# guoyihonggyh/MOBODY-Model-Based-Off-Dynamics-Offline-Reinforcement-Learning

Hardware: AMD Instinct MI355X
Metric: transitions/sec (minibatch rows through train(), refresh amortised at 1/5000) + grad-steps/sec (higher is better)
Workload: dtype f16x2

## Files before the change

### mobody-model-based-off-dynamics-offline-reinforcement-learning_amd/csrc/mlp_bwd.hip

```cpp
#include <stdlib.h>

#include "common.h"
#include "layers_bf.h"
#include "train.h"

namespace mobody {

template <int MT, int MASK>
struct MaskPre {
  uint32_t w[MASK == 1 ? MT : 1][2];
  float v[MASK == 1 ? 1 : MT][2][MASK == 1 ? 1 : 16];
};
template <int MT, int MASK>
__device__ __forceinline__ void mask_fetch(MaskPre<MT, MASK>& p, const float* __restrict__ h, const uint32_t* __restrict__ bits,
                                           int rows_here) {
  const int lane = lane_id(), w = wave_id(), i = lane & 31, hh = lane >> 5;
  if constexpr (MASK == 1) {
#pragma unroll
    for (int mt = 0; mt < MT; ++mt) {
      const int g = min(mt, (rows_here + 31) / 32 - 1);
      p.w[mt][0] = bits[g * HID + 64 * w + i]; p.w[mt][1] = bits[g * HID + 64 * w + 32 + i];
    }
  } else {
    const float* hp = h + 64 * w + i;
// ... 4 lines not shown
        const int row = min(32 * mt + (r & 3) + 8 * (r >> 2) + 4 * hh, rows_here - 1);
        p.v[mt][0][r] = hp[row * HID];
        p.v[mt][1][r] = hp[row * HID + 32];
      }
  }
}

template <int MT, int MASK>
__device__ __forceinline__ float wide_mask_apply(f32x16 (&acc)[MT][2], const MaskPre<MT, MASK>& pre, int rows_here, float prescale) {
  const int hh = lane_id() >> 5;
  constexpr bool BITS = MASK == 1;
  const auto& hv = pre.v;
  const auto& mw = pre.w;
  float mx = 0.f;
  f32x16 pa[MT][2];
#pragma unroll
  for (int mt = 0; mt < MT; ++mt) { pa[mt][0] = acc[mt][0] * prescale; pa[mt][1] = acc[mt][1] * prescale; }
  auto sweep = [&](auto guarded) {
#pragma unroll
    for (int mt = 0; mt < MT; ++mt)
#pragma unroll
      for (int nt = 0; nt < 2; ++nt)
#pragma unroll
        for (int r = 0; r < 16; ++r) {
          const int rb = (r & 3) + 8 * (r >> 2) + 4 * hh;
          const bool valid = !decltype(guarded)::value || 32 * mt + rb < rows_here;
          const float a = pa[mt][nt][r];
          float dz;
          if constexpr (MASK == 2) {
            dz = valid ? a * hv[mt][nt][r] : 0.f;
          } else {
            bool on;
            if constexpr (BITS) on = (mw[mt][nt] >> rb) & 1u;
            else on = hv[mt][nt][r] > 0.f;
            dz = (on && valid) ? a : 0.f;
          }
          acc[mt][nt][r] = dz;
          mx = fmaxf(mx, fabsf(dz));
        }
  };
  if (rows_here == 32 * MT) sweep(std::false_type{});
  else sweep(std::true_type{});
  return finite_tile_max<MT>(acc, mx);
}

template <int MT, int PM>
__device__ __forceinline__ void wide_store_colsum(f32x16 (&acc)[MT][2], float* Xs, float* gdst, int rows_here, int e,
                                                  float (&cs)[2], const PlaneSave& gs = PlaneSave{nullptr, 0, nullptr}) {
  const int lane = lane_id(), w = wave_id();
  const int i = lane & 31, hh = lane >> 5;
  cs[0] = cs[1] = 0.f;
  if constexpr (PM > 0) {
    const float sc = Split<PM>::F16 ? exp2i(e) : 1.f;
    if (gs.base != nullptr && (int)threadIdx.x < MT) gs.e_out[threadIdx.x] = e;
#pragma unroll
    for (int mt = 0; mt < MT; ++mt)
#pragma unroll
      for (int nt = 0; nt < 2; ++nt) {
        const f32x16 ys = Split<PM>::F16 ? acc[mt][nt] * sc : acc[mt][nt];
#pragma unroll
        for (int g = 0; g < 4; ++g) {
          float y4[4];
#pragma unroll
          for (int j = 0; j < 4; ++j) y4[j] = ys[4 * g + j];
          planes_store4<PM, 32 * MT>(reinterpret_cast<char*>(Xs), 64 * w + 32 * nt + i, 8 * mt + 2 * g + hh, y4, gs.base, gs.plane_stride);
        }
      }
  }
#pragma unroll
  for (int mt = 0; mt < MT; ++mt)
#pragma unroll
    for (int nt = 0; nt < 2; ++nt)
#pragma unroll
      for (int r = 0; r < 16; ++r) {
        const float dz = acc[mt][nt][r];
        if constexpr (PM == 0) Xs[(32 * mt + (r & 3) + 8 * (r >> 2) + 4 * hh) * LDX + 64 * w + 32 * nt + i] = dz;
        cs[nt] += dz;
      }
  if (gdst != nullptr) wide_store_rows<MT>(acc, gdst, rows_here);
  cs[0] += __shfl_xor(cs[0], 32);
  cs[1] += __shfl_xor(cs[1], 32);
}

__device__ __forceinline__ void bwd_seed(const Mlp3BwdArgs& a, float* Xs, float* red, int m, long long row0, int rows_here,
                                         int TB) {
  const BwdSeed& sd = a.seed;
  const int Np3 = a.Np3;
  const int t = threadIdx.x;
  float l0 = 0.f, l1 = 0.f;
  if (sd.mode == 1 || sd.mode == 2) {
    if (t < TB) {
      const bool ok = t < rows_here;
      const long long row = row0 + (ok ? t : 0);
      float v = 0.f;
      if (sd.mode == 1) {
        const float qn = sd.qnext ? sd.qnext[row] : fminf(sd.qt[row], sd.qt[a.rows + row]);
        const float y = sd.r[row] + sd.nd[row] * sd.gamma * qn;
        const float d = sd.q[(long long)m * a.rows + row] - y;
        v = ok ? 2.f * d * sd.inv_ng : 0.f;
        l0 = ok ? d * d : 0.f;
      } else {
        const ActorRowArgs& r = sd.ar;
        const float q0 = r.qp[row], q1 = r.qp[r.N + row];
        const float c = -policy_weight(r) / (float)r.Ng;
        const float g0 = q0 < q1 ? 1.f : (q0 == q1 ? 0.5f : 0.f);
        v = ok ? c * (m == 0 ? g0 : 1.f - g0) : 0.f;
        if (m == 0 && ok && row < r.Nt) r.bcw[row] = bc_weight(r, row);
      }
      Xs[t] = v;
      if (sd.dz3_out != nullptr && ok) {
        float* g = sd.dz3_out + ((long long)m * a.rows + row) * Np3;
        g[0] = v;
        for (int c = 1; c < Np3; ++c) g[c] = 0.f;
      }
    }
  } else {
    const ActorRowArgs& r = sd.ar;
    const float wscale = r.h.bc_coef * 2.f / ((float)r.Ntg * (float)r.A);
    for (int e = t; e < TB * Np3; e += NTHREADS) {
      const int rr = e / Np3, j = e - rr * Np3;
      const bool ok = rr < rows_here && j < r.A;
      const long long row = row0 + (rr < rows_here ? rr : 0);
      const int jc = j < r.A ? j : 0;
      const bool bc = row < r.Nt;
      const float p = r.pi[row * r.A + jc];
      const float d0 = r.dxa[row * r.A + jc], d1 = r.dxa[(r.N + row) * r.A + jc];
      const float act = r.act[row * r.A + jc];
      const float w = r.bcw[bc ? row : 0];
      float v = 0.f;
      if (ok) {
        float d = d0 + d1;
        if (bc) { const float df = p - act; d += wscale * w * df; l1 += w * (df * df); }
        const float th = p / r.h.max_action;
        v = d * r.h.max_action * (1.f - th * th);
        if (j == 0) l0 = l0 - fminf(r.qp[row], r.qp[r.N + row]);
      }
      Xs[rr * LDX + j] = v;
      if (rr < rows_here) sd.dz3_out[(row0 + rr) * Np3 + j] = v;
    }
  }
  if (sd.mode == 2) return;
#pragma unroll
  for (int o = 32; o > 0; o >>= 1) { l0 += __shfl_xor(l0, o); l1 += __shfl_xor(l1, o); }
  if ((t & 63) == 0) { red[t >> 6] = l0; red[4 + (t >> 6)] = l1; }
  lds_barrier();
  if (t == 0) {
    l0 = red[0] + red[1] + red[2] + red[3];
    l1 = red[4] + red[5] + red[6] + red[7];
    if (sd.mode == 1) sd.lossp[blockIdx.x * 2 + m] = l0;
    else { sd.lossp[2 * blockIdx.x] = l0; sd.lossp[2 * blockIdx.x + 1] = l1; }
  }
}

template <bool DX, int NT, int MASK, int PM = 0>
__global__ __launch_bounds__(NTHREADS, MASK == 1 ? 3 : 2) void k_mlp3_bwd(Mlp3BwdArgs a) {
  constexpr bool BITS = MASK == 1;
  __shared__ float red[8];
  extern __shared__ __attribute__((aligned(16))) float Xs[];
  constexpr int TB = MLP_TILE_ROWS, MT = MLP_MT;
  constexpr int PMX = PM > 0 ? PM : 1;
  const int m = blockIdx.y;
  const long long row0 = (long long)blockIdx.x * TB;
  const int rows_here = (int)min((long long)TB, a.rows - row0);
  const int lane = lane_id(), w = wave_id();
  const float* w3t = a.wt + m * a.t_mstride + a.w3t;
  const float* w2t = a.wt + m * a.t_mstride + a.w2t;
  const float* w1t = a.wt + m * a.t_mstride + a.w1t;
  const float* h1 = BITS ? nullptr : a.h1 + ((long long)m * a.rows + row0) * HID;
  const float* h2 = BITS ? nullptr : a.h2 + ((long long)m * a.rows + row0) * HID;
  const long long mtile = ((long long)m * cdiv(a.rows, 32) + row0 / 32) * HID;
  const uint32_t* m1 = BITS ? a.m1 + mtile : nullptr;
  const uint32_t* m2 = BITS ? a.m2 + mtile : nullptr;
  float* dz2 = a.dz2 ? a.dz2 + ((long long)m * a.rows + row0) * HID : nullptr;
  float* dz1 = a.dz1 ? a.dz1 + ((long long)m * a.rows + row0) * HID : nullptr;
  float* dbp = a.dbp + ((long long)blockIdx.x * gridDim.y + m) * (2 * HID + a.Np3);
  float* scr = reinterpret_cast<float*>(reinterpret_cast<char*>(Xs) + split_scr_offset<PMX, TB>());

  TR(0);
  MaskPre<MT, MASK> mk1, mk2;
  mask_fetch<MT, MASK>(mk2, h2, m2, rows_here);
  if constexpr (BITS) mask_fetch<MT, MASK>(mk1, h1, m1, rows_here);
  WideRingT<(PM > 0 ? 3 : WIDE_RING)> ring;
  const int mode = a.seed.mode;
  const bool rank1 = mode == 1 || mode == 2, with_db = mode != 2;
  const int c0 = (64 * w + (lane & 31)) * 4;
  const float w3c[2] = {w3t[c0], w3t[c0 + 128]};
  if (!rank1) wide_prefetch(w3t, a.Np3, ring);
  if (mode == 0) tile_load(Xs, 0, a.dz3 + ((long long)m * a.rows + row0) * a.Np3, a.Np3, a.Np3, 0, rows_here, TB);
  else bwd_seed(a, Xs, red, m, row0, rows_here, TB);
  lds_barrier();
  TR(1);
  if (with_db && (int)threadIdx.x < a.Np3) {
    float s = 0.f;
    if (!rank1) for (int r = 0; r < TB; ++r) s += Xs[r * LDX + threadIdx.x];
    else if (threadIdx.x == 0) for (int r = 0; r < TB; ++r) s += Xs[r];
    dbp[2 * HID + threadIdx.x] = s;
  }

  f32x16 acc[MT][2];
  float cs[2];
  if (rank1) {
    const int hh = lane >> 5;
#pragma unroll
    for (int mt = 0; mt < MT; ++mt)
#pragma unroll
      for (int g = 0; g < 4; ++g) {
        const f32x4 sv = *reinterpret_cast<const f32x4*>(Xs + 32 * mt + 8 * g + 4 * hh);
#pragma unroll
        for (int j = 0; j < 4; ++j) { acc[mt][0][4 * g + j] = sv[j] * w3c[0]; acc[mt][1][4 * g + j] = sv[j] * w3c[1]; }
      }
  } else {
    wide_zero<MT>(acc);
    wide_gemm<MT>(Xs, w3t, a.Np3, acc, ring);
  }
  TR(2);
  BfRing<PMX> bring;
  const s16x8* w2tp = PM > 0 ? reinterpret_cast<const s16x8*>(a.w2t_planes + m * a.planes_ms) : nullptr;
  if constexpr (PM > 0) bf_prefetch<PMX>(w2tp, bring);
  else wide_prefetch(w2t, HID, ring);
  int e2 = 0;
  {
    const float mx = wide_mask_apply<MT, MASK>(acc, mk2, rows_here, 1.f);
    if constexpr (PM == 4) f16_tile_max_put(mx, scr);
  }
  lds_barrier();
  if constexpr (PM == 4) e2 = f16_scale_exp(f16_tile_max_get(scr));
  PlaneSave gs{nullptr, 0, nullptr};
  if (PM == 4 && a.dz2p != nullptr) {
    gs.base = reinterpret_cast<short*>(a.dz2p) + m * a.dz2p_ms + (row0 / 8) * (HID * 8);
    gs.plane_stride = a.dz2p_plane;
    gs.e_out = a.e2_out + (long long)m * cdiv(a.rows, 32) + row0 / 32;
  }
  wide_store_colsum<MT, PM>(acc, Xs, dz2, rows_here, e2, cs, gs);
  if (with_db && lane < 32) { dbp[HID + 64 * w + lane] = cs[0]; dbp[HID + 64 * w + 32 + lane] = cs[1]; }
  lds_barrier();
  TR(3);
  if constexpr (!BITS) mask_fetch<MT, MASK>(mk1, h1, m1, rows_here);
  wide_zero<MT>(acc);
  if constexpr (PM > 0) bf_gemm<MT, PMX, TB>(reinterpret_cast<const char*>(Xs), w2tp, acc, bring);
  else wide_gemm<MT>(Xs, w2t, HID, acc, ring);
  TR(4);
  NarrowRegs<(NT > 0 ? NT : 1)> br;
  if constexpr (DX && NT > 0) narrow_prefetch<NT>(w1t, 16 * NT, br);
  wide_mask_apply<MT, MASK>(acc, mk1, rows_here, PM == 4 ? exp2i(-(e2 + F16_WSHIFT)) : 1.f);
  lds_barrier();
  wide_store_colsum<MT, 0>(acc, Xs, dz1, rows_here, 0, cs);
  if (with_db && lane < 32) { dbp[64 * w + lane] = cs[0]; dbp[64 * w + 32 + lane] = cs[1]; }
  TR(5);
  if constexpr (DX) {
    lds_barrier();
    float* dx = a.dx + ((long long)m * a.rows + row0) * a.dx_n;
    auto emit = [&](int row, int col, float v) {
      const int c = col - a.dx_c0;
      if (row < rows_here && c >= 0 && c < a.dx_n) dx[row * a.dx_n + c] = v;
    };
    if constexpr (NT > 0) narrow_run<TB / 16, NT>(Xs, br, emit);
    else narrow_layer(Xs, w1t, HID, a.Np1t, emit, TB);
  }
  TR(6);
}

template <bool DX, int NT, int BITS, int NPL = 0>
static int launch_bwd_t(const Mlp3BwdArgs& a, int members, hipStream_t st) {
  constexpr size_t lds = split_lds_bytes<(NPL > 0 ? NPL : 1), MLP_TILE_ROWS>();
  static bool once = false;
  if (!once) {
    int rc = allow_big_lds(k_mlp3_bwd<DX, NT, BITS, NPL>, lds);
    if (rc) return rc;
    once = true;
  }
  dim3 grid((unsigned)cdiv(a.rows, MLP_TILE_ROWS), (unsigned)members);
  ProfScope prof(PROF_MLP_BWD, st);
  hipLaunchKernelGGL((k_mlp3_bwd<DX, NT, BITS, NPL>), grid, dim3(NTHREADS), lds, st, a);
  MB_LAUNCH_OK("k_mlp3_bwd");
  return 0;
}

template <int NPL>
static int launch_bwd_bf(const Mlp3BwdArgs& a, int members, bool with_dx, hipStream_t st) {
  const int nt = a.Np1t == 16 ? 1 : a.Np1t == 32 ? 2 : 0;
  if (!with_dx) return launch_bwd_t<false, 0, 1, NPL>(a, members, st);
  return nt == 1 ? launch_bwd_t<true, 1, 1, NPL>(a, members, st) : nt == 2 ? launch_bwd_t<true, 2, 1, NPL>(a, members, st)
                                                                             : launch_bwd_t<true, 0, 1, NPL>(a, members, st);
}

template <int BITS>
static int launch_bwd_masks(const Mlp3BwdArgs& a, int members, bool with_dx, hipStream_t st) {
  const int nt = a.Np1t == 16 ? 1 : a.Np1t == 32 ? 2 : 0;
  if (!with_dx) return launch_bwd_t<false, 0, BITS>(a, members, st);
  return nt == 1 ? launch_bwd_t<true, 1, BITS>(a, members, st) : nt == 2 ? launch_bwd_t<true, 2, BITS>(a, members, st)
                                                                          : launch_bwd_t<true, 0, BITS>(a, members, st);
}

static int launch_bwd_swish(const Mlp3BwdArgs& a, int members, bool with_dx, hipStream_t st) {
  const int nt = a.Np1t == 16 ? 1 : a.Np1t == 32 ? 2 : 0;
  if (a.prec == PREC_F16X2 && a.w2t_planes != nullptr) {
    if (!with_dx) return launch_bwd_t<false, 0, 2, 4>(a, members, st);
    return nt == 1 ? launch_bwd_t<true, 1, 2, 4>(a, members, st) : nt == 2 ? launch_bwd_t<true, 2, 2, 4>(a, members, st)
                                                                             : launch_bwd_t<true, 0, 2, 4>(a, members, st);
  }
  if (!with_dx) return launch_bwd_t<false, 0, 2>(a, members, st);
  return nt == 1 ? launch_bwd_t<true, 1, 2>(a, members, st) : nt == 2 ? launch_bwd_t<true, 2, 2>(a, members, st)
                                                                         : launch_bwd_t<true, 0, 2>(a, members, st);
}

int launch_mlp3_bwd(const Mlp3BwdArgs& a, int members, bool with_dx, hipStream_t st) {
  if (a.rows <= 0) return 0;
  if (a.swish) return launch_bwd_swish(a, members, with_dx, st);
  if (a.prec != PREC_F32 && a.w2t_planes != nullptr && a.m1 != nullptr && a.m2 != nullptr)
    return a.prec == PREC_BF16 ? launch_bwd_bf<1>(a, members, with_dx, st) : a.prec == PREC_BF16X2 ? launch_bwd_bf<2>(a, members, with_dx, st)
         : a.prec == PREC_BF16X3 ? launch_bwd_bf<3>(a, members, with_dx, st) : launch_bwd_bf<4>(a, members, with_dx, st);
  return a.m1 != nullptr && a.m2 != nullptr ? launch_bwd_masks<1>(a, members, with_dx, st)
                                            : launch_bwd_masks<0>(a, members, with_dx, st);
}

__device__ __forceinline__ __amdgpu_buffer_rsrc_t slice_rsrc(const float* p, int nrows, int ld) {
  return __builtin_amdgcn_make_buffer_rsrc(const_cast<float*>(p), 0, (int)((unsigned)nrows * (unsigned)ld * 4u), 0x00020000);
}
__device__ __forceinline__ float buf_ld(__amdgpu_buffer_rsrc_t r, unsigned voff, unsigned soff) {
  return __builtin_bit_cast(float, __builtin_amdgcn_raw_buffer_load_b32(r, (int)voff, (int)soff, 0));
}

template <int MT, int NT>
__device__ __forceinline__ void wgrad_store(const WgradJob& jb, const WgradArgs& a, f32x16 (&acc)[MT][NT], int k0, int n0,
                                            int slice, int m, float* red) {
  constexpr int TK = 32 * MT, TN = 32 * NT;
  const int lane = lane_id(), w = wave_id();
  const int i = lane & 31, h = lane >> 5;
  float* mine = red + (w & 1) * (TK * TN);
  auto sweep = [&](bool add) {
#pragma unroll
    for (int x = 0; x < MT; ++x)
#pragma unroll
      for (int y = 0; y < NT; ++y)
#pragma unroll
        for (int r = 0; r < 16; ++r) {
          const int kk = 32 * x + (r & 3) + 8 * (r >> 2) + 4 * h;
          float* p = mine + kk * TN + 32 * y + i;
          *p = add ? *p + acc[x][y][r] : acc[x][y][r];
        }
  };
  if (w < 2) sweep(false);
  lds_barrier();
  if (w >= 2) sweep(true);
  lds_barrier();
  float* slab = a.slabs + (long long)slice * a.slab_stride + jb.out_off + m * a.out_mstride;
  if ((jb.wide || jb.transposed) && (jb.out_k & 3) == 0 && (!jb.transposed || (jb.out_ld & 3) == 0)) {
    for (int g = threadIdx.x; g < (TK / 4) * TN; g += NTHREADS) {
      const int kg = g / TN, nn = g - kg * TN;
      f32x4 s;
#pragma unroll
      for (int c = 0; c < 4; ++c) { const int idx = (4 * kg + c) * TN + nn; s[c] = red[idx] + red[TK * TN + idx]; }
      const int gk = k0 + 4 * kg, gn = n0 + nn;
      if (gk < jb.out_k && gn < jb.out_n)
        *reinterpret_cast<f32x4*>(slab + (jb.transposed ? (long long)gn * jb.out_ld + gk : wide_idx(gk, gn))) = s;
    }
    return;
  }
  for (int idx = threadIdx.x; idx < TK * TN; idx += NTHREADS) {
    const int kk = idx / TN, nn = idx - kk * TN;
    const float s = red[idx] + red[TK * TN + idx];
    const int gk = k0 + kk, gn = n0 + nn;
    if (gk < jb.out_k && gn < jb.out_n) {
      if (jb.transposed) slab[(long long)gn * jb.out_ld + gk] = s;
      else if (jb.wide) slab[wide_idx(gk, gn)] = s;
      else slab[(long long)gk * jb.out_ld + gn] = s;
    }
  }
}

template <int MT>
__device__ __forceinline__ void wgrad_tile(const WgradJob& jb, const WgradArgs& a, int tile, int slice, int m, float* red) {
  constexpr int NT = 2, TK = 32 * MT, TN = 32 * NT, U = 4, RB = 2 * U;
  const int lane = lane_id(), w = __builtin_amdgcn_readfirstlane(wave_id());
  const int i = lane & 31, h = lane >> 5;
  const int tk = tile / jb.tiles_n, tn = tile - tk * jb.tiles_n;
  const int k0 = tk * TK, n0 = tn * TN;
  const long long r_begin = ((long long)slice * 4 + w) * a.rows_per_wave;
  const long long r_end = min(a.rows, r_begin + a.rows_per_wave);
  const int lda = jb.lda, ldb = jb.ldb;

  f32x16 acc[MT][NT];
#pragma unroll
  for (int x = 0; x < MT; ++x)
#pragma unroll
    for (int y = 0; y < NT; ++y)
#pragma unroll
      for (int r = 0; r < 16; ++r) acc[x][y][r] = 0.f;

  unsigned oa[MT], ob[NT];
#pragma unroll
  for (int x = 0; x < MT; ++x) { const int c = k0 + 32 * x + i; oa[x] = 4u * (unsigned)((c < jb.ka ? c : 0) + h * lda); }
#pragma unroll
  for (int y = 0; y < NT; ++y) { const int c = n0 + 32 * y + i; ob[y] = 4u * (unsigned)((c < jb.nb ? c : 0) + h * ldb); }

  auto mma = [&](float (&av)[U][MT], float (&bv)[U][NT]) {
// ... 424 lines not shown
```

### mobody-model-based-off-dynamics-offline-reinforcement-learning_amd/csrc/train.h

```cpp
#pragma once
#include <math.h>
#include <stdlib.h>

#include "common.h"
#include "tile.h"
#include "tile_bf.h"
#include "health.h"

namespace mobody {

struct ActorRowArgs {
  const float *qp, *qb, *stats, *pi, *act, *dxa;
  const float* v_true;
  float* bcw;
  long long N, Nt, Ng, Ntg;
  int A;
  MobodyHyper h;
};
__device__ __forceinline__ float policy_weight(const ActorRowArgs& a) {
  return a.h.scale_q ? a.h.weight / (a.stats[0] / (float)a.Ng) : 1.f;
}
__device__ __forceinline__ float bc_weight(const ActorRowArgs& a, long long row) {
  if (!a.h.q_weighted) return 1.f;
  const float qb = fminf(a.qb[row], a.qb[a.Nt + row]);
  const float adv = a.v_true ? qb - a.v_true[row]
                             : qb / (a.stats[1] / (float)a.Ntg);
  return fminf(expf(3.f * adv), 100.f);
}

struct BwdSeed {
  int mode;
  const float *q, *qt, *qnext, *r, *nd;
  float gamma, inv_ng;
  ActorRowArgs ar;
  float* dz3_out;
  float* lossp;
};

struct Mlp3BwdArgs {
  BwdSeed seed;
  const float* dz3;
  const float* h1;
  const float* h2;
  int swish;
  const uint32_t* m1;
  const uint32_t* m2;
  const float* wt;
  const unsigned short* w2t_planes;
  long long planes_ms;
  int prec;
  long long t_mstride, w3t, w2t, w1t;
  int Np3, Np1t;
  long long rows;
  float* dz2;
  float* dz1;
  unsigned short* dz2p;
  long long dz2p_ms;
  long long dz2p_plane;
  int* e2_out;
  float* dbp;
  float* dx;
  int dx_c0, dx_n;
};
int launch_mlp3_bwd(const Mlp3BwdArgs& a, int members, bool with_dx, hipStream_t st);

inline Mlp3BwdArgs bwd_net(const MobodyMlpLayout& L, const float* blob_T, long long rows) {
  Mlp3BwdArgs b{};
  b.wt = blob_T; b.t_mstride = L.t_member_floats;
  b.w3t = L.w3t; b.w2t = L.w2t; b.w1t = L.w1t; b.Np3 = L.Np3; b.Np1t = L.Np1t; b.rows = rows;
  return b;
}
inline void bwd_set_planes(Mlp3BwdArgs& b, const MobodyMlpLayout& L, int prec) {
  b.prec = prec; b.w2t_planes = reinterpret_cast<const unsigned short*>(b.wt + L.w2tp); b.planes_ms = 2 * L.t_member_floats;
}
inline void bwd_set_acts(Mlp3BwdArgs& b, const float* h1, const float* h2, const uint32_t* m1, const uint32_t* m2, int swish) {
  b.h1 = h1; b.h2 = h2; b.m1 = m1; b.m2 = m2; b.swish = swish;
}
inline void bwd_set_grads(Mlp3BwdArgs& b, const float* dz3, float* dz2, float* dz1, float* dbp, int* e2 = nullptr) {
  if (e2 != nullptr && dz2 != nullptr) {
    const long long r32 = (b.rows + 31) & ~31LL;
    b.dz2p = reinterpret_cast<unsigned short*>(dz2); b.dz2p_plane = r32 * HID; b.dz2p_ms = 2 * r32 * HID; b.e2_out = e2;
    dz2 = nullptr;
  }
  b.dz3 = dz3; b.dz2 = dz2; b.dz1 = dz1; b.dbp = dbp;
}

struct WgradJob {
  const float* A; long long a_mstride; int lda, ka;
  const float* B; long long b_mstride; int ldb, nb;
  long long out_off; int out_ld, out_k, out_n;
  int transposed;
  int wide;
  int tiles_n, ntiles;
};
struct WgradArgs {
  const int *eA, *eB;
  long long e_mstride, plane_stride;
  WgradJob job[3];
  long long rows, rows_per_wave;
  float* slabs; long long slab_stride, out_mstride;
  int nsplit, members, tiles_total;
  float* bc_out; const long long* bc_t; float bc_lr;
  int prec;
};
int launch_wgrad(WgradArgs a, hipStream_t st);

struct AdamConsts { float step_size, bc2_sqrt, tau, one_minus_tau, gscale; };
constexpr float ADAM_W1 = (float)(1.0 - 0.9), ADAM_B2 = (float)0.999, ADAM_W2 = (float)(1.0 - 0.999), ADAM_EPS = 1e-8f;

__device__ __forceinline__ void write_w2_planes(float* t_member, const MobodyMlpLayout& L, int k, int n, float w, int precision) {
  short* p2 = reinterpret_cast<short*>(t_member + L.w2p);
  short* p2t = reinterpret_cast<short*>(t_member + L.w2tp);
  if (precision == 4) {
    short t[2];
    split_terms<4>(w * exp2i(F16_WSHIFT), t);
#pragma unroll
    for (int p = 0; p < 2; ++p) { p2[bf_plane_idx(p, k, n)] = t[p]; p2t[bf_plane_idx(p, n, k)] = t[p]; }
  } else {
    short t[3];
    split_terms<3>(w, t);
#pragma unroll
    for (int p = 0; p < 3; ++p) { p2[bf_plane_idx(p, k, n)] = t[p]; p2t[bf_plane_idx(p, n, k)] = t[p]; }
  }
}

__device__ __forceinline__ long long t_blob_index(const MobodyMlpLayout& L, long long o) {
  if (o < L.b1) {
    const long long g = o >> 2;
    const int k = (int)(g / HID) * 4 + (int)(o & 3), n = (int)(g % HID);
    return L.w1t + (long long)n * L.Np1t + k;
  }
  if (o >= L.w2 && o < L.b2) {
    const long long oo = o - L.w2, g = oo >> 2;
    const int k = (int)(g / HID) * 4 + (int)(oo & 3), n = (int)(g % HID);
    return L.w2t + wide_idx(n, k);
  }
  if (o >= L.w3 && o < L.b3) {
    const long long oo = o - L.w3;
    const int k = (int)(oo / L.Np3), n3 = (int)(oo % L.Np3);
    return L.w3t + wide_idx(n3, k);
  }
  return -1;
}

struct AdamTarget {
  float *p, *m, *v, *target, *blob_T;
  float* target_T;
// ... 129 lines not shown
```

### mobody-model-based-off-dynamics-offline-reinforcement-learning_amd/csrc/train.hip

```cpp
#include <math.h>

#include "common.h"
#include "layers.h"
#include "train.h"

namespace mobody {

struct TrainWs {
  uint32_t *mq1, *mq2, *ma1, *ma2;
  int *eh1q, *eh1a, *edz2;
  float *pin;
  float *pi, *qt, *q, *qb, *xq, *h1q, *h2q, *xa, *h1a, *h2a, *dz3q, *dz2, *dz1, *dz3a, *dxa, *bcw, *dbp, *slabs, *lossp;
  float *bc;
  long long total;
  int nsplit_q, nsplit_a, ntiles;
  MobodyMlpLayout Lq, La;
};

static int carve(const MobodyTrainDims& d, float* base, TrainWs& w) {
  int rc = mobody_mlp_layout(d.S + d.A, 1, 2, &w.Lq);
  if (rc) return rc;
  rc = mobody_mlp_layout(d.S, d.A, 1, &w.La);
  if (rc) return rc;
  const long long N = d.N, Nt = d.Nt;
  const long long N32 = (N + 31) & ~31LL;
  long long off = 0;
  auto take = [&](long long n) { float* p = base ? base + off : nullptr; off += (n + 3) & ~3LL; return p; };
  w.pi = take(N * d.A);
  w.pin = take(N * d.A);
  w.qt = take(2 * N);
  w.q = take(2 * N);
  w.qb = take(2 * Nt);
  w.xq = take(N * w.Lq.Kp1);
  w.h1q = take(2 * N32 * HID);
  w.h2q = take(2 * N * HID);
  w.xa = take(N * w.La.Kp1);
  w.h1a = take(N32 * HID);
  w.h2a = take(N * HID);
  const long long mw = cdiv(N, 32) * HID;
  w.mq1 = (uint32_t*)take(2 * mw); w.mq2 = (uint32_t*)take(2 * mw);
  w.ma1 = (uint32_t*)take(mw); w.ma2 = (uint32_t*)take(mw);
  w.eh1q = (int*)take(2 * (N32 / 32)); w.eh1a = (int*)take(N32 / 32); w.edz2 = (int*)take(2 * (N32 / 32));
  w.dz3q = take(2 * N * w.Lq.Np3);
  w.dz2 = take(2 * N32 * HID);
  w.dz1 = take(2 * N * HID);
  w.dz3a = take(N * w.La.Np3);
  w.dxa = take(2 * N * d.A);
  w.bcw = take(Nt > 0 ? Nt : 1);
  w.lossp = take(2 * cdiv(N, 32));
  w.ntiles = (int)cdiv(N, MLP_TILE_ROWS);
  w.nsplit_q = wgrad_nsplit(N, 2);
  w.nsplit_a = wgrad_nsplit(N, 1);
  const long long per_q = 2 * HID + w.Lq.Np3, per_a = 2 * HID + w.La.Np3;
  w.dbp = take((long long)w.ntiles * (2 * per_q > per_a ? 2 * per_q : per_a));
  {
    const long long sq = ((w.Lq.total_floats + 3) & ~3LL) * w.nsplit_q, sa = ((w.La.total_floats + 3) & ~3LL) * w.nsplit_a;
    w.slabs = take(sq > sa ? sq : sa);
  }
  w.bc = take(4);
  w.total = off;
  return 0;
}

static int check_dims(const MobodyTrainDims* d, const char* who) {
  MB_REQUIRE(d != nullptr, "%s: dims is null", who);
  MB_REQUIRE(d->N >= 1 && d->Nt >= 0 && d->Nt <= d->N, "%s: need 1 <= N and 0 <= Nt <= N (N=%lld Nt=%lld)", who,
             (long long)d->N, (long long)d->Nt);
  MB_REQUIRE(d->N_global >= d->N && d->Nt_global >= d->Nt, "%s: global row counts smaller than local", who);
  return 0;
}

__device__ __forceinline__ float block_sum(float v, float* sm) {
#pragma unroll
  for (int o = 32; o > 0; o >>= 1) v += __shfl_xor(v, o);
  const int w = threadIdx.x >> 6, nw = blockDim.x >> 6;
  __syncthreads();
  if ((threadIdx.x & 63) == 0) sm[w] = v;
  __syncthreads();
  float s = 0.f;
  for (int k = 0; k < nw; ++k) s += sm[k];
  return s;
}

__global__ __launch_bounds__(1024) void k_actor_stats(const float* qp, const float* qb, long long N, long long Nt,
                                                      float* stats) {
  __shared__ float sm[16];
  constexpr int U = 4;
  float s0 = 0.f, s1 = 0.f;
  for (long long base = threadIdx.x; base < N; base += U * 1024) {
    float a[U], b[U];
#pragma unroll
    for (int u = 0; u < U; ++u) { const long long r = base + u * 1024; const long long rc = r < N ? r : 0; a[u] = qp[rc]; b[u] = qp[N + rc]; }
#pragma unroll
    for (int u = 0; u < U; ++u) if (base + u * 1024 < N) s0 += fabsf(fminf(a[u], b[u]));
  }
  for (long long base = threadIdx.x; base < Nt; base += U * 1024) {
    float a[U], b[U];
#pragma unroll
    for (int u = 0; u < U; ++u) { const long long r = base + u * 1024; const long long rc = r < Nt ? r : 0; a[u] = qb[rc]; b[u] = qb[Nt + rc]; }
#pragma unroll
    for (int u = 0; u < U; ++u) if (base + u * 1024 < Nt) s1 += fabsf(fminf(a[u], b[u]));
  }
  s0 = block_sum(s0, sm);
  s1 = block_sum(s1, sm);
  if (threadIdx.x == 0) { stats[0] = s0; stats[1] = s1; }
}

__global__ __launch_bounds__(256) void k_v_loss(const float* qt, const float* v, long long N, float invNg, int Np3,
                                                float* dz3, float* lossp) {
  __shared__ float sm[4];
  const long long row = (long long)blockIdx.x * blockDim.x + threadIdx.x;
  float l = 0.f;
  if (row < N) {
    const float adv = fminf(qt[row], qt[N + row]) - v[row];
    const float w = fabsf(0.7f - (adv < 0.f ? 1.f : 0.f));
    l = w * adv * adv;
    float* o = dz3 + row * Np3;
    o[0] = -2.f * w * adv * invNg;
    for (int c = 1; c < Np3; ++c) o[c] = 0.f;
  }
  l = block_sum(l, sm);
  if (threadIdx.x == 0) lossp[blockIdx.x] = l;
}
__global__ __launch_bounds__(256) void k_sum_scale(const float* parts, int n, float scale, float* out) {
  __shared__ float sm[4];
  float s = 0.f;
  for (int k = threadIdx.x; k < n; k += blockDim.x) s += parts[k];
  s = block_sum(s, sm);
  if (threadIdx.x == 0) out[0] = s * scale;
}

__global__ __launch_bounds__(256) void k_adam(AdamTarget a, const float* g, long long n, MobodyMlpLayout L) {
  __shared__ float adam_sm[2];
  adam_block_consts(a, adam_sm);
  const long long j = (long long)blockIdx.x * blockDim.x + threadIdx.x;
  if (j >= n || (health_mask(a) != 0 && health_foreign(a))) return;
  adam_element(a, L, j, g[j], adam_sm);
}

int launch_adam(const AdamTarget& a, const float* g, const MobodyMlpLayout& L, hipStream_t st) {
  hipLaunchKernelGGL(k_adam, dim3((unsigned)cdiv(L.total_floats, 256)), dim3(256), 0, st, a, g, (long long)L.total_floats, L);
  MB_LAUNCH_OK("k_adam");
  return 0;
}

__global__ __launch_bounds__(256) void k_mlp_transpose(MobodyMlpLayout L, const float* blob, float* bt, int precision, int* health) {
  const long long j = (long long)blockIdx.x * blockDim.x + threadIdx.x;
  if (j >= L.t_total_floats) return;
  const int m = (int)(j / L.t_member_floats);
  const long long o = j - (long long)m * L.t_member_floats;
  const float* src = blob + (long long)m * L.member_floats;
  if (o >= L.w2p) {
    if (o >= L.w2p + HID * HID) return;
    const int e = (int)(o - L.w2p), k = e / HID, n = e % HID;
    const float w = src[L.w2 + wide_idx(k, n)];
    write_w2_planes(bt + (long long)m * L.t_member_floats, L, k, n, w, precision);
    if (precision == 4) {
      short* tm = reinterpret_cast<short*>(bt + (long long)m * L.t_member_floats);
      tm[2 * L.w2p + bf_plane_idx(2, k, n)] = 0; tm[2 * L.w2tp + bf_plane_idx(2, n, k)] = 0;
      health_check_f16(health, w);
    }
    return;
  }
  float val;
  if (o < L.w1t) {
    const bool is3 = o < L.w2t;
    const long long oo = is3 ? o : o - L.w2t;
    const long long g = oo >> 2;
    const int kk = (int)(g / HID) * 4 + (int)(oo & 3), c = (int)(g % HID);
// ... 85 lines not shown
                                  prec == PREC_F16X2 ? w.eh1q : nullptr);
  if (a.phase == 2) {
  } else if (q_next == nullptr) {
    const Mlp3FwdArgs fpn = fwd_args(a.actor_blob, w.La, next_state, S, nullptr, 0, N, w.pin, 1, h->max_action, nullptr, nullptr, nullptr, nullptr, nullptr, aT);
    if (gather != nullptr) {
      FwdGather fg = *gather;
      fwd_set_gather(fg, 0, fq, 0);
      fwd_set_gather(fg, 1, fpn, S + A);
      rc = launch_mlp3_forward_gather(fq, 2, fpn, 1, fg, prec, st);
    } else {
      rc = launch_mlp3_forward(fq, 2, fpn, 1, ACT_RELU, prec, st);
    }
    const Mlp3FwdArgs ft = fwd_args(a.qtarg_blob, w.Lq, next_state, S, w.pin, A, N, w.qt, 0, 1.f, nullptr, nullptr, nullptr, nullptr, nullptr, tT);
    if (!rc && a.policy_forward)
      rc = launch_mlp3_forward(ft, 2, fwd_args(a.actor_blob, w.La, state, S, nullptr, 0, N, w.pi, 1, h->max_action, w.xa, w.h1a, w.h2a, w.ma1, w.ma2, aT,
                                               prec == PREC_F16X2 ? w.eh1a : nullptr), 1, ACT_RELU, prec, st);
    else if (!rc)
      rc = launch_mlp3_forward(ft, 2, ACT_RELU, prec, st);
  } else {
    rc = launch_mlp3_forward(fq, 2, ACT_RELU, prec, st);
  }
  if (rc || a.phase == 1) return rc;
  const float invNg = 1.f / (float)d->N_global;
  Mlp3BwdArgs bq = bwd_args(w.Lq, a.q_blob_T, w.dz3q, w.h1q, w.h2q, N, w.dz2, w.dz1, w.dbp, w.mq1, w.mq2, prec, w.edz2);
  bq.seed.mode = 1; bq.seed.q = w.q; bq.seed.qt = w.qt; bq.seed.qnext = q_next; bq.seed.r = a.reward; bq.seed.nd = a.not_done;
  bq.seed.gamma = h->gamma; bq.seed.inv_ng = invNg; bq.seed.dz3_out = w.dz3q; bq.seed.lossp = w.lossp;
  rc = launch_mlp3_bwd(bq, 2, false, st);
  if (rc) return rc;
  LossFinal lf{};
  lf.kind = 1; lf.nparts = 2 * w.ntiles; lf.scale = invNg; lf.parts = w.lossp; lf.out = a.loss_out;
  return weight_grads(w.Lq, w.xq, w.h1q, w.h2q, w.dz3q, w.dz2, w.dz1, N, w, a.grad_q, lf, adam, st, prec, w.eh1q);
}

extern "C" int mobody_critic(const MobodyCritic* a, void* stream) {
  const char* who = "mobody_critic";
  MB_BLOCK(who, a, MobodyCritic);
  MB_REQUIRE((a->grad_q != nullptr) != (a->m != nullptr || a->v != nullptr), "%s: exactly one of grad_q and the optimizer state m, v must be given", who);
  MB_REQUIRE(a->grad_q || (a->m && a->v), "%s: null pointer", who);
  MB_REQUIRE(a->phase >= 0 && a->phase <= 2, "%s: phase is 0 (the whole step), 1 (forwards) or 2 (backward + update)", who);
  if (a->gather == nullptr) return critic_impl(*a, nullptr, stream);
  const MobodyGatherRng* gr = a->gather;
  MB_REQUIRE(a->phase == 0, "%s: the step cannot be split (phase %d): the first forward launch writes the minibatch the backward reads", who, a->phase);
  MB_REQUIRE(a->q_next == nullptr, "%s: q_next given: the launch that gathers is the one that evaluates pi(s')", who);
  FwdGather fg{};
  long long N;
  int rc = gather_args_rng(who, fg.g, gr->bufs, gr->counts, gr->nbuf, a->d.S, a->d.A, gr->seeds, gr->call_offsets, gr->counter, gr->sizes,
                           a->state, a->action, a->next_state, a->reward, a->not_done, gr->bump, gr->nbump, N);
  if (rc) return rc;
  MB_REQUIRE(N == a->d.N, "%s: the counts add up to %lld rows, the step runs on %lld", who, N, (long long)a->d.N);
  for (int k = 0; k < gr->nbuf; ++k)
    MB_REQUIRE(gr->counts[k] == 0 || fg.g.packed[k], "%s: source %d is not a row-interleaved ring (mobody_ring_pitch)", who, k);
  return critic_impl(*a, &fg, stream);
}

extern "C" int mobody_actor_forward(const MobodyActor* a, void* stream) {
  const char* who = "mobody_actor_forward";
  MB_BLOCK(who, a, MobodyActor);
  const MobodyTrainDims* d = &a->d;
  const MobodyHyper* h = &a->h;
  int rc = check_dims(d, who);
  if (rc) return rc;
  MB_REQUIRE(a->actor_blob && a->q_blob && a->state && a->action && a->stats && a->workspace, "%s: null pointer", who);
  rc = check_precision(who, h->precision, a->actor_blob_T && a->q_blob_T);
  if (rc) return rc;
  const int prec = h->precision;
  const float *aT = prec != PREC_F32 ? a->actor_blob_T : nullptr, *qT = prec != PREC_F32 ? a->q_blob_T : nullptr;
  const float *q_blob = a->q_blob, *state = a->state;
  TrainWs w;
  rc = carve(*d, a->workspace, w);
  if (rc) return rc;
  hipStream_t st = as_stream(stream);
  const long long N = d->N, Nt = d->Nt;
  const int S = d->S, A = d->A;
  const Mlp3FwdArgs fb = fwd_args(q_blob, w.Lq, state, S, a->action, A, Nt, w.qb, 0, 1.f, nullptr, nullptr, nullptr, nullptr, nullptr, qT);
  const Mlp3FwdArgs fp = fwd_args(q_blob, w.Lq, state, S, w.pi, A, N, w.q, 0, 1.f, nullptr, nullptr, nullptr, w.mq1, w.mq2, qT);
  if (a->policy_ready) {
    rc = launch_mlp3_forward(fb, 2, fp, 2, ACT_RELU, prec, st);
  } else {
    rc = launch_mlp3_forward(fb, 2, fwd_args(a->actor_blob, w.La, state, S, nullptr, 0, N, w.pi, 1, h->max_action, w.xa, w.h1a, w.h2a, w.ma1, w.ma2, aT,
                                             prec == PREC_F16X2 ? w.eh1a : nullptr), 1, ACT_RELU, prec, st);
    if (!rc) rc = launch_mlp3_forward(fp, 2, ACT_RELU, prec, st);
  }
  if (rc) return rc;
  hipLaunchKernelGGL(k_actor_stats, dim3(1), dim3(1024), 0, st, w.q, w.qb, N, Nt, a->stats);
  MB_LAUNCH_OK("k_actor_stats");
  return 0;
}

static int actor_backward_impl(const MobodyActor& a, void* stream) {
  const char* who = "mobody_actor_backward";
  const MobodyTrainDims* d = &a.d;
  const MobodyHyper* h = &a.h;
  const bool fused = a.m != nullptr;
  int rc = check_dims(d, who);
  if (rc) return rc;
  MB_REQUIRE(a.actor_blob && a.actor_blob_T && a.q_blob && a.q_blob_T && a.state && a.action && a.stats && a.loss_out && a.workspace,
             "%s: null pointer", who);
  rc = check_precision(who, h->precision, true);
  if (rc) return rc;
  MB_REQUIRE(!fused || a.t_dev != nullptr || a.t >= 1, "%s: step t must be >= 1", who);
  TrainWs w;
  rc = carve(*d, a.workspace, w);
  if (rc) return rc;
  const AdamTarget adam = fused ? adam_target(a.actor_blob, a.actor_blob_T, a.m, a.v, nullptr, a.t, a.t_dev, a.lr, -1.f, 1.f, h->precision) : AdamTarget{};
  hipStream_t st = as_stream(stream);
  const long long N = d->N;
  ActorRowArgs ra{};
  ra.qp = w.q; ra.qb = w.qb; ra.stats = a.stats; ra.pi = w.pi; ra.act = a.action; ra.dxa = w.dxa; ra.v_true = a.v_true;
  ra.bcw = w.bcw; ra.N = N; ra.Nt = d->Nt; ra.Ng = d->N_global; ra.Ntg = d->Nt_global > 0 ? d->Nt_global : 1;
  ra.A = d->A; ra.h = *h;
  Mlp3BwdArgs bq = bwd_args(w.Lq, a.q_blob_T, nullptr, nullptr, nullptr, N, nullptr, nullptr, w.dbp, w.mq1, w.mq2, h->precision);
  bq.seed.mode = 2; bq.seed.ar = ra;
  bq.dx = w.dxa; bq.dx_c0 = d->S; bq.dx_n = d->A;
  rc = launch_mlp3_bwd(bq, 2, true, st);
  if (rc) return rc;
  Mlp3BwdArgs ba = bwd_args(w.La, a.actor_blob_T, w.dz3a, w.h1a, w.h2a, N, w.dz2, w.dz1, w.dbp, w.ma1, w.ma2, h->precision, w.edz2);
  ba.seed.mode = 3; ba.seed.ar = ra; ba.seed.dz3_out = w.dz3a; ba.seed.lossp = w.lossp;
  rc = launch_mlp3_bwd(ba, 1, false, st);
  if (rc) return rc;
  LossFinal lf{};
  lf.kind = 2; lf.nparts = w.ntiles; lf.scale_q = h->scale_q; lf.weight = h->weight; lf.bc_coef = h->bc_coef;
  lf.ng = (float)ra.Ng; lf.ntg_a = (float)ra.Ntg * (float)ra.A; lf.parts = w.lossp; lf.stats = a.stats; lf.out = a.loss_out;
  return weight_grads(w.La, w.xa, w.h1a, w.h2a, w.dz3a, w.dz2, w.dz1, N, w, a.grad_actor, lf, adam, st, h->precision, w.eh1a);
}

extern "C" int mobody_actor_backward(const MobodyActor* a, void* stream) {
  const char* who = "mobody_actor_backward";
  MB_BLOCK(who, a, MobodyActor);
  MB_REQUIRE((a->grad_actor != nullptr) != (a->m != nullptr || a->v != nullptr), "%s: exactly one of grad_actor and the optimizer state m, v must be given", who);
  MB_REQUIRE(a->grad_actor || (a->m && a->v), "%s: null pointer", who);
  return actor_backward_impl(*a, stream);
}

extern "C" int mobody_mlp_transpose(int in_dim, int out_dim, int members, const float* blob, float* blob_T, int precision,
                                    void* stream) {
  MobodyMlpLayout L;
  int rc = mobody_mlp_layout(in_dim, out_dim, members, &L);
  if (rc) return rc;
  MB_REQUIRE(blob && blob_T, "mobody_mlp_transpose: null pointer");
  rc = check_precision("mobody_mlp_transpose", precision, true);
  if (rc) return rc;
  hipLaunchKernelGGL(k_mlp_transpose, dim3((unsigned)cdiv(L.t_total_floats, 256)), dim3(256), 0, as_stream(stream), L, blob, blob_T,
                     precision, health_words());
  MB_LAUNCH_OK("k_mlp_transpose");
  return 0;
}

static int adam_impl(const MobodyAdam& a, void* stream) {
  const char* who = "mobody_adam_polyak";
  MobodyMlpLayout L;
  int rc = mobody_mlp_layout(a.in_dim, a.out_dim, a.members, &L);
  if (rc) return rc;
  MB_REQUIRE(a.blob && a.grad && a.m && a.v, "%s: null pointer", who);
  MB_REQUIRE(a.t_dev != nullptr || a.t >= 1, "%s: step t must be >= 1", who);
  rc = check_precision(who, a.precision, true);
  if (rc) return rc;
  AdamTarget at = adam_target(a.blob, a.blob_T, a.m, a.v, a.target, a.t, a.t_dev, a.lr, a.tau, a.grad_scale, a.precision);
  at.target_T = at.target ? a.target_T : nullptr;
  hipStream_t st = as_stream(stream);
  hipLaunchKernelGGL(k_adam, dim3((unsigned)cdiv(L.total_floats, 256)), dim3(256), 0, st, at, a.grad, (long long)L.total_floats, L);
  MB_LAUNCH_OK("k_adam");
  return 0;
}

extern "C" int mobody_adam_polyak(const MobodyAdam* a, void* stream) {
  MB_BLOCK("mobody_adam_polyak", a, MobodyAdam);
  return adam_impl(*a, stream);
}

namespace mobody {
__global__ __launch_bounds__(256) void k_par_penalty(const float* ns_true, const float* ns_model, float* reward, float coef,
                                                     long long n, int S) {
  const long long row = (long long)blockIdx.x * blockDim.x + threadIdx.x;
  if (row >= n) return;
  double s = 0.0;
  for (int d = 0; d < S; ++d) { const double e = (double)ns_true[row * S + d] - (double)ns_model[row * S + d]; s += e * e; }
  reward[row] = (float)((double)reward[row] - (double)coef * (s / (double)S));
}
}

extern "C" int mobody_par_penalty(const float* next_state_true, const float* next_state_model, float* reward, float coef,
                                  int64_t n, int S, void* stream) {
  MB_REQUIRE(n >= 0 && S >= 1, "mobody_par_penalty: bad sizes");
  if (n == 0) return 0;
  MB_REQUIRE(next_state_true && next_state_model && reward, "mobody_par_penalty: null pointer");
  hipLaunchKernelGGL(k_par_penalty, dim3((unsigned)cdiv(n, 256)), dim3(256), 0, as_stream(stream), next_state_true,
                     next_state_model, reward, coef, (long long)n, S);
  MB_LAUNCH_OK("k_par_penalty");
  return 0;
}


extern "C" int mobody_value_loss_grad(const float* qt, const float* v, int64_t N, int64_t N_global, float* dz3,
                                      float* loss_out, float* lossp_ws, void* stream) {
  MB_REQUIRE(N >= 1 && N_global >= N, "mobody_value_loss_grad: bad sizes");
  MB_REQUIRE(qt && v && dz3 && loss_out && lossp_ws, "mobody_value_loss_grad: null pointer");
  const int nb = (int)cdiv(N, 256);
  const float invNg = 1.f / (float)N_global;
  hipStream_t st = as_stream(stream);
  hipLaunchKernelGGL(k_v_loss, dim3(nb), dim3(256), 0, st, qt, v, (long long)N, invNg, 16, dz3, lossp_ws);
  MB_LAUNCH_OK("k_v_loss");
// ... 5 lines not shown
```

Baseline: 50.06 million.

## Chain actor Q-backward and policy-backward in one kernel via per-tile tickets

Fuses the two actor backward launches (critic pass producing dx for actions, then actor MLP pass) into one kernel. Each tile's two critic-member blocks bump a per-tile atomic ticket, and the last one to finish runs the actor backward for that tile, reading dxa and bcw through agent-scope atomic loads. This removes a kernel launch and the full-grid dependency barrier so the actor pass can overlap with the remaining critic tiles. Tickets are reset in the stats kernel. The seed loop is also unrolled to batch loads. Half the blocks do extra serial work, and correctness relies on memory ordering with relaxed atomics and on kernarg layout tricks.

```diff
diff --git a/mobody-model-based-off-dynamics-offline-reinforcement-learning_amd/csrc/mlp_bwd.hip b/mobody-model-based-off-dynamics-offline-reinforcement-learning_amd/csrc/mlp_bwd.hip
--- a/mobody-model-based-off-dynamics-offline-reinforcement-learning_amd/csrc/mlp_bwd.hip
+++ b/mobody-model-based-off-dynamics-offline-reinforcement-learning_amd/csrc/mlp_bwd.hip
@@ -110,8 +110,11 @@
   cs[1] += __shfl_xor(cs[1], 32);
 }
 
-__device__ __forceinline__ void bwd_seed(const Mlp3BwdArgs& a, float* Xs, float* red, int m, long long row0, int rows_here,
-                                         int TB) {
+__device__ __forceinline__ void agent_store(float* p, float v) { __hip_atomic_store(p, v, __ATOMIC_RELAXED, __HIP_MEMORY_SCOPE_AGENT); }
+__device__ __forceinline__ float agent_load(const float* p) { return __hip_atomic_load(p, __ATOMIC_RELAXED, __HIP_MEMORY_SCOPE_AGENT); }
+template <bool CHAIN = false>
+__device__ __forceinline__ void bwd_seed(const Mlp3BwdArgs& a, float* Xs, float* red, int m, int tile, long long row0,
+                                         int rows_here, int TB) {
   const BwdSeed& sd = a.seed;
   const int Np3 = a.Np3;
   const int t = threadIdx.x;
@@ -133,7 +136,10 @@
         const float c = -policy_weight(r) / (float)r.Ng;
         const float g0 = q0 < q1 ? 1.f : (q0 == q1 ? 0.5f : 0.f);
         v = ok ? c * (m == 0 ? g0 : 1.f - g0) : 0.f;
-        if (m == 0 && ok && row < r.Nt) r.bcw[row] = bc_weight(r, row);
+        if (m == 0 && ok && row < r.Nt) {
+          if constexpr (CHAIN) agent_store(r.bcw + row, bc_weight(r, row));
+          else r.bcw[row] = bc_weight(r, row);
+        }
       }
       Xs[t] = v;
       if (sd.dz3_out != nullptr && ok) {
@@ -145,6 +151,7 @@
   } else {
     const ActorRowArgs& r = sd.ar;
     const float wscale = r.h.bc_coef * 2.f / ((float)r.Ntg * (float)r.A);
+    if constexpr (!CHAIN) {
     for (int e = t; e < TB * Np3; e += NTHREADS) {
       const int rr = e / Np3, j = e - rr * Np3;
       const bool ok = rr < rows_here && j < r.A;
@@ -166,6 +173,45 @@
       Xs[rr * LDX + j] = v;
       if (rr < rows_here) sd.dz3_out[(row0 + rr) * Np3 + j] = v;
     }
+    } else {
+    constexpr int SEED_U = 4;
+    for (int e0 = t; e0 < TB * Np3; e0 += SEED_U * NTHREADS) {
+      float pv[SEED_U], d0v[SEED_U], d1v[SEED_U], av[SEED_U], wv[SEED_U], qv[SEED_U][2];
+#pragma unroll
+      for (int u = 0; u < SEED_U; ++u) {
+        const int e = min(e0 + u * NTHREADS, TB * Np3 - 1);
+        const int rr = e / Np3, j = e - rr * Np3;
+        const long long row = row0 + (rr < rows_here ? rr : 0);
+        const int jc = j < r.A ? j : 0;
+        const float* dp = r.dxa + row * r.A + jc;
+        pv[u] = r.pi[row * r.A + jc]; av[u] = r.act[row * r.A + jc];
+        qv[u][0] = r.qp[row]; qv[u][1] = r.qp[r.N + row];
+        d0v[u] = agent_load(dp); d1v[u] = agent_load(dp + r.N * r.A);
+        wv[u] = agent_load(row < r.Nt ? r.bcw + row : dp);
+      }
+#pragma unroll
+      for (int u = 0; u < SEED_U; ++u) {
+        const int e = e0 + u * NTHREADS;
+        if (e < TB * Np3) {
+          const int rr = e / Np3, j = e - rr * Np3;
+          const bool ok = rr < rows_here && j < r.A;
+          const long long row = row0 + (rr < rows_here ? rr : 0);
+          const bool bc = row < r.Nt;
+          const float p = pv[u], w = wv[u];
+          float v = 0.f;
+          if (ok) {
+            float d = d0v[u] + d1v[u];
+            if (bc) { const float df = p - av[u]; d += wscale * w * df; l1 += w * (df * df); }
+            const float th = p / r.h.max_action;
+            v = d * r.h.max_action * (1.f - th * th);
+            if (j == 0) l0 = l0 - fminf(qv[u][0], qv[u][1]);
+          }
+          Xs[rr * LDX + j] = v;
+          if (rr < rows_here) sd.dz3_out[(row0 + rr) * Np3 + j] = v;
+        }
+      }
+    }
+    }
   }
   if (sd.mode == 2) return;
 #pragma unroll
@@ -175,20 +221,17 @@
   if (t == 0) {
     l0 = red[0] + red[1] + red[2] + red[3];
     l1 = red[4] + red[5] + red[6] + red[7];
-    if (sd.mode == 1) sd.lossp[blockIdx.x * 2 + m] = l0;
-    else { sd.lossp[2 * blockIdx.x] = l0; sd.lossp[2 * blockIdx.x + 1] = l1; }
-  }
-}
-
-template <bool DX, int NT, int MASK, int PM = 0>
-__global__ __launch_bounds__(NTHREADS, MASK == 1 ? 3 : 2) void k_mlp3_bwd(Mlp3BwdArgs a) {
+    if (sd.mode == 1) sd.lossp[tile * 2 + m] = l0;
+    else { sd.lossp[2 * tile] = l0; sd.lossp[2 * tile + 1] = l1; }
+  }
+}
+
+template <bool DX, int NT, int MASK, int PM = 0, bool CHAIN = false>
+__device__ __forceinline__ void mlp3_bwd_tile(const Mlp3BwdArgs& a, int m, int tile, int members, float* Xs, float* red) {
   constexpr bool BITS = MASK == 1;
-  __shared__ float red[8];
-  extern __shared__ __attribute__((aligned(16))) float Xs[];
   constexpr int TB = MLP_TILE_ROWS, MT = MLP_MT;
   constexpr int PMX = PM > 0 ? PM : 1;
-  const int m = blockIdx.y;
-  const long long row0 = (long long)blockIdx.x * TB;
+  const long long row0 = (long long)tile * TB;
   const int rows_here = (int)min((long long)TB, a.rows - row0);
   const int lane = lane_id(), w = wave_id();
   const float* w3t = a.wt + m * a.t_mstride + a.w3t;
@@ -201,7 +244,7 @@
   const uint32_t* m2 = BITS ? a.m2 + mtile : nullptr;
   float* dz2 = a.dz2 ? a.dz2 + ((long long)m * a.rows + row0) * HID : nullptr;
   float* dz1 = a.dz1 ? a.dz1 + ((long long)m * a.rows + row0) * HID : nullptr;
-  float* dbp = a.dbp + ((long long)blockIdx.x * gridDim.y + m) * (2 * HID + a.Np3);
+  float* dbp = a.dbp + ((long long)tile * members + m) * (2 * HID + a.Np3);
   float* scr = reinterpret_cast<float*>(reinterpret_cast<char*>(Xs) + split_scr_offset<PMX, TB>());
 
   TR(0);
@@ -215,7 +258,7 @@
   const float w3c[2] = {w3t[c0], w3t[c0 + 128]};
   if (!rank1) wide_prefetch(w3t, a.Np3, ring);
   if (mode == 0) tile_load(Xs, 0, a.dz3 + ((long long)m * a.rows + row0) * a.Np3, a.Np3, a.Np3, 0, rows_here, TB);
-  else bwd_seed(a, Xs, red, m, row0, rows_here, TB);
+  else bwd_seed<CHAIN>(a, Xs, red, m, tile, row0, rows_here, TB);
   lds_barrier();
   TR(1);
   if (with_db && (int)threadIdx.x < a.Np3) {
@@ -280,12 +323,22 @@
     float* dx = a.dx + ((long long)m * a.rows + row0) * a.dx_n;
     auto emit = [&](int row, int col, float v) {
       const int c = col - a.dx_c0;
-      if (row < rows_here && c >= 0 && c < a.dx_n) dx[row * a.dx_n + c] = v;
+      if (row < rows_here && c >= 0 && c < a.dx_n) {
+        if constexpr (CHAIN) agent_store(dx + row * a.dx_n + c, v);
+        else dx[row * a.dx_n + c] = v;
+      }
     };
     if constexpr (NT > 0) narrow_run<TB / 16, NT>(Xs, br, emit);
     else narrow_layer(Xs, w1t, HID, a.Np1t, emit, TB);
   }
   TR(6);
+}
+
+template <bool DX, int NT, int MASK, int PM = 0>
+__global__ __launch_bounds__(NTHREADS, MASK == 1 ? 3 : 2) void k_mlp3_bwd(Mlp3BwdArgs a) {
+  __shared__ float red[8];
+  extern __shared__ __attribute__((aligned(16))) float Xs[];
+  mlp3_bwd_tile<DX, NT, MASK, PM>(a, blockIdx.y, blockIdx.x, gridDim.y, Xs, red);
 }
 
 template <bool DX, int NT, int BITS, int NPL = 0>
@@ -340,6 +393,63 @@
          : a.prec == PREC_BF16X3 ? launch_bwd_bf<3>(a, members, with_dx, st) : launch_bwd_bf<4>(a, members, with_dx, st);
   return a.m1 != nullptr && a.m2 != nullptr ? launch_bwd_masks<1>(a, members, with_dx, st)
                                             : launch_bwd_masks<0>(a, members, with_dx, st);
+}
+
+template <int NT, int PM>
+__global__ __launch_bounds__(NTHREADS, 3) void k_actor_bwd_chain(Mlp3BwdArgs q, Mlp3BwdArgs pi, int* tickets) {
+  __shared__ float red[8];
+  extern __shared__ __attribute__((aligned(16))) float Xs[];
+  const int tile = blockIdx.x;
+  mlp3_bwd_tile<true, NT, 1, PM, true>(q, blockIdx.y, tile, 2, Xs, red);
+  asm volatile("s_waitcnt vmcnt(0)" ::: "memory");
+  __syncthreads();
+  if (threadIdx.x == 0) {
+    const int t = __hip_atomic_fetch_add(tickets + tile, 1, __ATOMIC_RELAXED, __HIP_MEMORY_SCOPE_AGENT);
+    if (t == 1) __hip_atomic_store(tickets + tile, 0, __ATOMIC_RELAXED, __HIP_MEMORY_SCOPE_AGENT);
+    red[0] = __int_as_float(t);
+  }
+  __syncthreads();
+  __builtin_amdgcn_fence(__ATOMIC_ACQUIRE, "wavefront");
+  const int ticket = __float_as_int(red[0]);
+  if (ticket != 1) return;
+  lds_barrier();
+  static_assert(sizeof(Mlp3BwdArgs) % 8 == 0 && alignof(Mlp3BwdArgs) == 8, "`pi` follows `q` in the kernel-argument segment");
+  using KernArg = const __attribute__((address_space(4))) Mlp3BwdArgs;
+  KernArg* ka = (KernArg*)__builtin_amdgcn_kernarg_segment_ptr() + 1;
+  asm volatile("" : "+s"(ka));
+  mlp3_bwd_tile<false, 0, 1, PM, true>(*(const Mlp3BwdArgs*)ka, 0, tile, 1, Xs, red);
+}
+
+template <int NT, int PM>
+static int launch_chain_t(const Mlp3BwdArgs& q, const Mlp3BwdArgs& pi, int* tickets, hipStream_t st) {
+  constexpr size_t lds = split_lds_bytes<(PM > 0 ? PM : 1), MLP_TILE_ROWS>();
+  static bool once = false;
+  if (!once) {
+    int rc = allow_big_lds(k_actor_bwd_chain<NT, PM>, lds);
+    if (rc) return rc;
+    once = true;
+  }
+  dim3 grid((unsigned)cdiv(q.rows, MLP_TILE_ROWS), 2u);
+  ProfScope prof(PROF_MLP_BWD, st);
+  hipLaunchKernelGGL((k_actor_bwd_chain<NT, PM>), grid, dim3(NTHREADS), lds, st, q, pi, tickets);
+  MB_LAUNCH_OK("k_actor_bwd_chain");
+  return 0;
+}
+template <int PM>
+static int launch_chain_nt(const Mlp3BwdArgs& q, const Mlp3BwdArgs& pi, int* tickets, hipStream_t st) {
+  return q.Np1t == 16 ? launch_chain_t<1, PM>(q, pi, tickets, st) : q.Np1t == 32 ? launch_chain_t<2, PM>(q, pi, tickets, st)
+                                                                                   : launch_chain_t<0, PM>(q, pi, tickets, st);
+}
+
+int launch_actor_bwd_chain(const Mlp3BwdArgs& q, const Mlp3BwdArgs& pi, int* tickets, hipStream_t st) {
+  if (q.rows <= 0) return 0;
+  MB_REQUIRE(q.seed.mode == 2 && pi.seed.mode == 3 && q.rows == pi.rows && q.prec == pi.prec && tickets != nullptr &&
+             q.m1 && q.m2 && pi.m1 && pi.m2 && !q.swish && !pi.swish && (q.w2t_planes != nullptr) == (pi.w2t_planes != nullptr),
+             "launch_actor_bwd_chain: the two passes do not form an actor update");
+  if (q.prec != PREC_F32 && q.w2t_planes != nullptr)
+    return q.prec == PREC_BF16 ? launch_chain_nt<1>(q, pi, tickets, st) : q.prec == PREC_BF16X2 ? launch_chain_nt<2>(q, pi, tickets, st)
+         : q.prec == PREC_BF16X3 ? launch_chain_nt<3>(q, pi, tickets, st) : launch_chain_nt<4>(q, pi, tickets, st);
+  return launch_chain_nt<0>(q, pi, tickets, st);
 }
 
 __device__ __forceinline__ __amdgpu_buffer_rsrc_t slice_rsrc(const float* p, int nrows, int ld) {
diff --git a/mobody-model-based-off-dynamics-offline-reinforcement-learning_amd/csrc/train.h b/mobody-model-based-off-dynamics-offline-reinforcement-learning_amd/csrc/train.h
--- a/mobody-model-based-off-dynamics-offline-reinforcement-learning_amd/csrc/train.h
+++ b/mobody-model-based-off-dynamics-offline-reinforcement-learning_amd/csrc/train.h
@@ -63,6 +63,7 @@
   int dx_c0, dx_n;
 };
 int launch_mlp3_bwd(const Mlp3BwdArgs& a, int members, bool with_dx, hipStream_t st);
+int launch_actor_bwd_chain(const Mlp3BwdArgs& q, const Mlp3BwdArgs& pi, int* tickets, hipStream_t st);
 
 inline Mlp3BwdArgs bwd_net(const MobodyMlpLayout& L, const float* blob_T, long long rows) {
   Mlp3BwdArgs b{};
diff --git a/mobody-model-based-off-dynamics-offline-reinforcement-learning_amd/csrc/train.hip b/mobody-model-based-off-dynamics-offline-reinforcement-learning_amd/csrc/train.hip
--- a/mobody-model-based-off-dynamics-offline-reinforcement-learning_amd/csrc/train.hip
+++ b/mobody-model-based-off-dynamics-offline-reinforcement-learning_amd/csrc/train.hip
@@ -12,6 +12,7 @@
   float *pin;
   float *pi, *qt, *q, *qb, *xq, *h1q, *h2q, *xa, *h1a, *h2a, *dz3q, *dz2, *dz1, *dz3a, *dxa, *bcw, *dbp, *slabs, *lossp;
   float *bc;
+  int *tickets;
   long long total;
   int nsplit_q, nsplit_a, ntiles;
   MobodyMlpLayout Lq, La;
@@ -58,6 +59,7 @@
     w.slabs = take(sq > sa ? sq : sa);
   }
   w.bc = take(4);
+  w.tickets = (int*)take(w.ntiles);
   w.total = off;
   return 0;
 }
@@ -83,8 +85,9 @@
 }
 
 __global__ __launch_bounds__(1024) void k_actor_stats(const float* qp, const float* qb, long long N, long long Nt,
-                                                      float* stats) {
+                                                      float* stats, int* tickets, int ntickets) {
   __shared__ float sm[16];
+  for (int k = threadIdx.x; k < ntickets; k += 1024) tickets[k] = 0;
   constexpr int U = 4;
   float s0 = 0.f, s1 = 0.f;
   for (long long base = threadIdx.x; base < N; base += U * 1024) {
@@ -336,7 +339,7 @@
     if (!rc) rc = launch_mlp3_forward(fp, 2, ACT_RELU, prec, st);
   }
   if (rc) return rc;
-  hipLaunchKernelGGL(k_actor_stats, dim3(1), dim3(1024), 0, st, w.q, w.qb, N, Nt, a->stats);
+  hipLaunchKernelGGL(k_actor_stats, dim3(1), dim3(1024), 0, st, w.q, w.qb, N, Nt, a->stats, w.tickets, w.ntiles);
   MB_LAUNCH_OK("k_actor_stats");
   return 0;
 }
@@ -366,11 +369,9 @@
   Mlp3BwdArgs bq = bwd_args(w.Lq, a.q_blob_T, nullptr, nullptr, nullptr, N, nullptr, nullptr, w.dbp, w.mq1, w.mq2, h->precision);
   bq.seed.mode = 2; bq.seed.ar = ra;
   bq.dx = w.dxa; bq.dx_c0 = d->S; bq.dx_n = d->A;
-  rc = launch_mlp3_bwd(bq, 2, true, st);
-  if (rc) return rc;
   Mlp3BwdArgs ba = bwd_args(w.La, a.actor_blob_T, w.dz3a, w.h1a, w.h2a, N, w.dz2, w.dz1, w.dbp, w.ma1, w.ma2, h->precision, w.edz2);
   ba.seed.mode = 3; ba.seed.ar = ra; ba.seed.dz3_out = w.dz3a; ba.seed.lossp = w.lossp;
-  rc = launch_mlp3_bwd(ba, 1, false, st);
+  rc = launch_actor_bwd_chain(bq, ba, w.tickets, st);
   if (rc) return rc;
   LossFinal lf{};
   lf.kind = 2; lf.nparts = w.ntiles; lf.scale_q = h->scale_q; lf.weight = h->weight; lf.bc_coef = h->bc_coef;
```

Measured after the change: 50.96 million (median of 6 runs). 1.8% higher.
